# christoskokas/gtsam-vSLAM

Measured on AMD Instinct MI355X. Metric: frames/sec (extract+match+localBA), 1500 feat stereo 752x480, higher is better.
Workload: dtype u8/i32 (extract, match) + f64 (pose LM, local BA)

## Files before the change

gtsam-vslam_amd/csrc/ba.hip:

```cpp
#include "common.hpp"
#include "comm.hpp"
#include "dmath.hpp"
#include "ba_pool.hpp"
#include <algorithm>
#include <cmath>
#include <numeric>
#include <vector>
#include <atomic>
#include <condition_variable>
#include <functional>
#include <memory>
#include <mutex>
#include <thread>

namespace vslam {

struct BaEdge {
    int a, b, fa, fb;
    DPose measured;
    double r[6], Ja[36], Jb[36];
    double Haa[36], Hab[36], Hbb[36], ga[6], gb[6];
};

struct BaDev {
// ... 41 lines not shown
    D.poseCur = D.poseBase + (size_t)sel * D.K; D.poseTrial = D.poseBase + (size_t)ts * D.K;
    D.lmCur = D.lmBase + (size_t)sel * D.lmStride; D.lmTrial = D.lmBase + (size_t)ts * D.lmStride;
    if (D.specLin) {
        const size_t se = (size_t)D.n * D.n + D.n;
        D.facJ = D.facJBase + (size_t)sel * D.facJStride; D.facJ2 = D.facJBase + (size_t)ts * D.facJStride;
        D.Sedge = D.SedgeBase + (size_t)sel * se; D.Sedge2 = D.SedgeBase + (size_t)ts * se;
        D.edges = D.edgesBase + (size_t)sel * D.NE; D.edges2 = D.edgesBase + (size_t)ts * D.NE;
    }
    D.S += (size_t)c * D.sysStride; D.rhs += (size_t)c * D.sysStride; D.Spart += (size_t)c * D.spartStride;
    D.dP += (size_t)c * D.n; D.dL += (size_t)c * D.dLStride; D.partial += (size_t)c * D.partialStride;
    double lam = D.ctl[CTL_LAMBDA];
    for (int i = 0; i < c; i++) lam *= 10.0;
    D.lambda = lam;
    return true;
}

constexpr int BA_SCHUR_WAVES = 16;
constexpr int BA_LDS_MAX_F = 20;
constexpr int BA_LDS_BYTES = 160 * 1024, BA_STATIC_LDS_RESERVE = 1024, BA_DYN_LDS_MAX = BA_LDS_BYTES - BA_STATIC_LDS_RESERVE;

__device__ __forceinline__ void ba_eval_fac(const BaDev& D, const DPose& T, const double* p, bool right,
                                            const double* z, double is, double* r, double* Jp, double* Jl) {
    const double d[3] = {p[0] - T.t[0], p[1] - T.t[1], p[2] - T.t[2]};
    double q[3];
    mat3T_vec(T.R, d, q);
    if (Jp) { for (int c = 0; c < 12; c++) Jp[c] = 0; for (int c = 0; c < 6; c++) Jl[c] = 0; }
    if (is == 0.0) { r[0] = r[1] = 0.0; return; }
    if (q[2] <= 0) { r[0] = r[1] = 2.0 * D.fx * is; return; }
    const double x = q[0], y = q[1], zz = q[2], iz = 1.0 / zz;
    const double xx = right ? x - D.b : x;
// ... 182 lines not shown
    ci[CI_NACT] = D.NB;
}

__global__ __launch_bounds__(256) void k_ba_ctl(const BaDev* __restrict__ tab, int mode, double relTol, double absTol) {
    BaDev D = *lane_entry(tab, blockIdx.z);
    __shared__ int sZero;
    if (threadIdx.x == 0) {
        ba_ctl(D, mode, relTol, absTol);
        sZero = mode == 1 && ((const int*)(D.ctl + CTL_INTS))[CI_STATE] == BA_LINEARIZE;
    }
    __syncthreads();
    if (sZero) for (int i = threadIdx.x; i < D.n * D.n + D.n; i += 256) D.Sedge[i] = 0;
}

template <int MODE>
__global__ __launch_bounds__(256) void k_ba_factors(const BaDev* __restrict__ tab, int obsBlocks, int fuseCtl, double relTol, double absTol) {
    BaDev D = *lane_entry(tab, blockIdx.z);
    __shared__ double red[8], out[2];
    __shared__ double sW[160];
    __shared__ int sLast;
    double* const partialBase = D.partial;
    const int cand = MODE == 0 ? 0 : (int)blockIdx.y;
    const bool active = ba_enter(D, MODE == 0 ? BA_LINEARIZE : BA_TRY, cand);
    if (!active && ((const int*)(D.ctl + CTL_INTS))[CI_STATE] != (MODE == 0 ? BA_LINEARIZE : BA_TRY)) return;
    const int tid = threadIdx.x;
    if (!active) {
    } else if ((int)blockIdx.x < obsBlocks) {
        double v[2] = {0, 0};
        for (int f = blockIdx.x * 256 + tid; f < D.NF; f += obsBlocks * 256) {
            if (MODE == 0) {
                double r[2], Jp[12], Jl[6];
                ba_eval_fac(D, D.poseCur[D.facKf[f]], D.lmCur + 3 * (size_t)D.facLm[f], D.facRight[f], D.facZ + 2 * (size_t)f,
                            D.facIs[f], r, Jp, Jl);
                double* o = D.facJ + (size_t)f * 20;
                o[0] = r[0]; o[1] = r[1];
                for (int c = 0; c < 12; c++) o[2 + c] = Jp[c];
                for (int c = 0; c < 6; c++) o[14 + c] = Jl[c];
                v[0] += r[0] * r[0] + r[1] * r[1];
            } else {
                const double* o = D.facJ + (size_t)f * 20;
                const int fi = D.facFi[f], lp = D.facLp[f];
                double l0 = o[0], l1 = o[1];
                if (fi >= 0) {
                    const double* dp = D.dP + 6 * fi;
// ... 6 lines not shown
                if (D.specLin) {
                    double Jp[12], Jl[6];
                    ba_eval_fac(D, D.poseTrial[D.facKf[f]], D.lmTrial + 3 * (size_t)D.facLm[f], D.facRight[f], D.facZ + 2 * (size_t)f,
                                D.facIs[f], r, Jp, Jl);
                    double* o2 = D.facJ2 + (size_t)f * 20;
                    o2[0] = r[0]; o2[1] = r[1];
                    for (int c = 0; c < 12; c++) o2[2 + c] = Jp[c];
                    for (int c = 0; c < 6; c++) o2[14 + c] = Jl[c];
                } else
                    ba_eval_fac(D, D.poseTrial[D.facKf[f]], D.lmTrial + 3 * (size_t)D.facLm[f], D.facRight[f], D.facZ + 2 * (size_t)f,
                                D.facIs[f], r, nullptr, nullptr);
                v[1] += r[0] * r[0] + r[1] * r[1];
            }
        }
        ba_block_sum<2, 4>(v, red, out);
        if (tid == 0) { ba_publish(&D.partial[2 * blockIdx.x], out[0]); ba_publish(&D.partial[2 * blockIdx.x + 1], out[1]); }
    } else {
        const int e = blockIdx.x - obsBlocks;
        double v[2] = {0, 0};
        if (e < D.NE) {
            const BaEdge& E = D.edges[e];
            const int fa = E.fa, fb = E.fb;
            if (MODE == 0) {
                v[0] = ba_edge_linearize(D.edges[e], E, D.poseCur[E.a], D.poseCur[E.b], sW, D.Sedge, D.n, tid);
            } else {
                if (tid >= 8 && tid < 14) {
                    const int k = tid - 8;
                    double l = E.r[k];
                    for (int i = 0; i < 6; i++) {
                        if (fa >= 0) l += E.Ja[k * 6 + i] * D.dP[6 * fa + i];
                        if (fb >= 0) l += E.Jb[k * 6 + i] * D.dP[6 * fb + i];
                    }
                    v[0] += l * l;
// ... 6 lines not shown
                    pose_inverse(E.measured, Mi);
                    pose_compose(Mi, h, d);
                    double r[6];
                    pose3_logmap(d, r);
                    for (int i = 0; i < 6; i++) { r[i] *= 1.0 / 0.01; v[1] += r[i] * r[i]; }
                }
            }
#pragma unroll
            for (int k = 0; k < 2; k++) {
#pragma unroll
                for (int d = 32; d >= 1; d >>= 1) v[k] += __shfl_xor(v[k], d);
            }
            if (tid == 0) { ba_publish(&D.partial[2 * obsBlocks + 2 * e], v[0]); ba_publish(&D.partial[2 * obsBlocks + 2 * e + 1], v[1]); }
        }
    }
    asm volatile("s_waitcnt vmcnt(0)" ::: "memory");
    __syncthreads();
    const int nCandRun = MODE == 0 ? 1 : D.nAct;
    if (tid == 0) sLast = (__hip_atomic_fetch_add(&D.flags[FLAG_COUNT], 1, __ATOMIC_RELAXED, __HIP_MEMORY_SCOPE_AGENT) == (int)(gridDim.x * gridDim.y) - 1);
    __syncthreads();
    if (!sLast) return;
    const int nPart = obsBlocks + D.NE;
    for (int c = 0; c < nCandRun; c++) {
        const double* part = partialBase + (size_t)c * D.partialStride;
        double t[2] = {0, 0};
        for (int i = tid; i < nPart; i += 256) { t[0] += ba_collect(&part[2 * i]); t[1] += ba_collect(&part[2 * i + 1]); }
        ba_block_sum<2, 4>(t, red, out);
        if (tid == 0) {
            if (MODE == 0) D.sums[0] = 0.5 * out[0];
            else { D.sums[SUMS_CAND + 2 * c] = 0.5 * out[0]; D.sums[SUMS_CAND + 2 * c + 1] = 0.5 * out[1]; }
        }
        __syncthreads();
    }
    if (tid == 0) {
        D.flags[FLAG_COUNT] = 0;
        sLast = 0;
        if (fuseCtl) {
            ba_ctl(D, MODE, relTol, absTol);
            sLast = MODE == 1 && !D.specLin && ((const int*)(D.ctl + CTL_INTS))[CI_STATE] == BA_LINEARIZE;
            if (D.ctlHost) {
                asm volatile("s_waitcnt vmcnt(0) lgkmcnt(0)" ::: "memory");
// ... 43 lines not shown
        double acc = 0;
        for (int f = D.slotStart[s0 + s]; f < D.slotStart[s0 + s + 1]; f++) {
            const double* o = D.facJ + (size_t)f * 20;
            acc += o[2 + i] * o[14 + j] + o[2 + 6 + i] * o[14 + 3 + j];
        }
        W[e] = acc;
    }
    for (int s = lane; s < ns; s += BA_LPL) sfi[s] = D.slotFi[s0 + s];
}
__device__ __forceinline__ void ba_hll_inverse(const double* h, double lambda, double* Hi) {
    const double Hll[9] = {h[0] + lambda, h[1], h[2], h[1], h[3] + lambda, h[4], h[2], h[4], h[5] + lambda};
    inv3sym(Hll, Hi);
}

__global__ __launch_bounds__(64 * BA_SCHUR_WAVES) void k_ba_schur(const BaDev* __restrict__ tab, int maxSlots, int sharedW) {
    BaDev D = *lane_entry(tab, blockIdx.z);
    constexpr bool LDS_S = true;
    extern __shared__ double sm[];
    double* const SBase = D.S;
    double* const SpartBase = D.Spart;
    (void)SBase;
    const int c0 = sharedW ? 0 : (int)blockIdx.y;
    if (!ba_enter(D, BA_TRY, c0)) return;
    const int nc = sharedW ? D.nAct : 1;
    const int n = D.n;
    const size_t sys = (size_t)n * n + n;
    constexpr int BA_LPL = BA_LPL_SCHUR;
    double* Sloc = sm;
    double* wbase = sm + (LDS_S ? (size_t)nc * sys : 0);
    static_assert(BA_LPL == 64, "one wave per landmark: the landmark index is wave-uniform");
    const int lane = threadIdx.x & (BA_LPL - 1);
    const int unit = __builtin_amdgcn_readfirstlane(threadIdx.x / BA_LPL);
    double* W = wbase + (size_t)unit * (2 * maxSlots * 18);
    double* WH = W + maxSlots * 18;
    const int nu = blockDim.x / BA_LPL, nt = blockDim.x;
    int* sfi = (int*)(wbase + (size_t)nu * (2 * maxSlots * 18)) + unit * maxSlots;
    if (LDS_S) {
        for (int i = threadIdx.x; i < (int)(nc * sys); i += nt) Sloc[i] = 0;
    }
    __syncthreads();
    const int bi = lane / 6, bj = lane - bi * 6;
    const bool isBlk = lane < 36, isRhs = lane >= 36 && lane < 42;
    const int rr = isRhs ? lane - 36 : 0;
    const int hHalf = lane >= 27 ? 1 : 0, hq = lane - 27 * hHalf;
    const bool hRhs = hq >= 21;
    int hI = 0, hJ = 0;
    if (hRhs) hI = hq - 21;
    else { int rem = hq; while (rem >= 6 - hI) { rem -= 6 - hI; hI++; } hJ = hI + rem; }
    const int rounds = (D.Lp + gridDim.x * nu - 1) / (gridDim.x * nu);
    for (int rd = 0; rd < rounds; rd++) {
        const int lp = (rd * gridDim.x + blockIdx.x) * nu + unit;
        const bool act = lp < D.Lp;
        double h[9];
        int ns = 0;
        ba_lm_blocks<BA_LPL>(D, lp, act, W, sfi, h, ns);
        ba_wave_fence();
        double lamk = D.lambda;
        for (int k = 0; k < nc; k++, lamk *= 10.0) {
            double* Sacc = LDS_S ? Sloc + (size_t)k * sys : SBase + (size_t)(c0 + k) * D.sysStride;
            double* racc = Sacc + (size_t)n * n;
            double Hi[9];
            ba_hll_inverse(h, lamk, Hi);
            for (int e = lane; e < ns * 18; e += BA_LPL) {
                const int s = e / 18, ij = e - s * 18, i = ij / 3, j = ij - i * 3;
                const double* w = W + s * 18 + i * 3;
                WH[e] = w[0] * Hi[j] + w[1] * Hi[3 + j] + w[2] * Hi[6 + j];
// ... 18 lines not shown
        const int f0 = act ? D.lpStart[lp] : 0, f1 = act ? D.lpStart[lp + 1] : 0;
        if (lane < 54) {
            for (int f = f0 + hHalf; f < f1; f += 2) {
                const int fi = D.facFi[f];
                if (fi < 0) continue;
                const double* o = D.facJ + (size_t)f * 20;
                const double val = hRhs ? -(o[2 + hI] * o[0] + o[8 + hI] * o[1]) : o[2 + hI] * o[2 + hJ] + o[8 + hI] * o[8 + hJ];
                const size_t idx = hRhs ? (size_t)n * n + 6 * fi + hI : (size_t)(6 * fi + hI) * n + 6 * fi + hJ;
                for (int k = 0; k < nc; k++) atomicAdd((LDS_S ? Sloc + (size_t)k * sys : SBase + (size_t)(c0 + k) * D.sysStride) + idx, val);
            }
        }
    }
    if (LDS_S) {
        __syncthreads();
        for (int k = 0; k < nc; k++) {
            double* dst = SpartBase + (size_t)(c0 + k) * D.spartStride + (size_t)blockIdx.x * sys;
            for (int i = threadIdx.x; i < (int)sys; i += nt) dst[i] = Sloc[(size_t)k * sys + i];
        }
    }
}

constexpr int BA2_MAX_F = 10;
__host__ __device__ inline int ba2_stage_doubles(int maxFac, int maxSlots) {
    const int ints = maxFac + 2 * (maxSlots + 1);
    return ((maxFac * 20 + 2 * maxSlots * 18 + 10 + (ints + 1) / 2) + 1) & ~1;
}
__device__ __forceinline__ double ba2_dpp_xor(double v, int which) {
    const int lo = __double2loint(v), hi = __double2hiint(v);
    int l2, h2;
    if (which == 0) { l2 = __builtin_amdgcn_update_dpp(0, lo, 0xB1, 0xF, 0xF, true); h2 = __builtin_amdgcn_update_dpp(0, hi, 0xB1, 0xF, 0xF, true); }
    else { l2 = __builtin_amdgcn_update_dpp(0, lo, 0x4E, 0xF, 0xF, true); h2 = __builtin_amdgcn_update_dpp(0, hi, 0x4E, 0xF, 0xF, true); }
    return __hiloint2double(h2, l2);
}
// ... 45 lines not shown
#pragma unroll
    for (int k = 0; k < 9; k++) h[k] = g.hb[k];
}
__device__ __forceinline__ void ba2_w_row(const Ba2Region& g, const Ba2Roles& R, double& w0, double& w1, double& w2) {
    w0 = w1 = w2 = 0;
    for (int f = g.sst[R.ws]; f < g.sst[R.ws + 1]; f++) {
        const double* o = g.F + f * 20;
        const double a0 = o[2 + R.wi], a1 = o[8 + R.wi];
        w0 += a0 * o[14] + a1 * o[17];
        w1 += a0 * o[15] + a1 * o[18];
        w2 += a0 * o[16] + a1 * o[19];
    }
}

__global__ __launch_bounds__(1024) void k_ba_schur2(const BaDev* __restrict__ tab, int maxSlots, int maxFac) {
    BaDev D = *lane_entry(tab, blockIdx.z);
    extern __shared__ double sm[];
    if (!ba_enter(D, BA_TRY, blockIdx.y)) return;
    const int n = D.n;
    const int sys = n * n + n;
    double* const Sloc = sm;
    double* const racc = Sloc + (size_t)n * n;
    const int lane = threadIdx.x & 63;
    const int unit = __builtin_amdgcn_readfirstlane(threadIdx.x >> 6), nu = blockDim.x >> 6, nt = blockDim.x;
    const Ba2Region g = ba2_region(sm + sys + (size_t)unit * ba2_stage_doubles(maxFac, maxSlots), maxFac, maxSlots);
    double* const F = g.F; double* const W = g.W; double* const WH = g.WH;
    int* const ffi = g.ffi; int* const sfi = g.sfi;
    const double lam = D.lambda;
    Ba2Roles R;
    R.init(lane);
    const int pf = lane / 6, pi = lane - pf * 6;
    for (int i = threadIdx.x; i < sys; i += nt) Sloc[i] = 0;
    __syncthreads();
    for (int lp = blockIdx.x * nu + unit; lp < D.Lp; lp += gridDim.x * nu) {
        double h[9];
        int nf, ns;
        ba2_stage_h(D, lp, g, R, lane, h, nf, ns);
        double Hi[9];
        ba_hll_inverse(h, lam, Hi);
        if (R.ws < ns) {
            double w0, w1, w2;
            ba2_w_row(g, R, w0, w1, w2);
            const double g0 = w0 * Hi[0] + w1 * Hi[3] + w2 * Hi[6], g1 = w0 * Hi[1] + w1 * Hi[4] + w2 * Hi[7], g2 = w0 * Hi[2] + w1 * Hi[5] + w2 * Hi[8];
            double* wr = W + R.ws * 18 + R.wi * 3;
            wr[0] = w0; wr[1] = w1; wr[2] = w2;
            double* gr = WH + R.ws * 18 + R.wi * 3;
            gr[0] = g0; gr[1] = g1; gr[2] = g2;
            atomicAdd(&racc[6 * sfi[R.ws] + R.wi], -(g0 * h[6] + g1 * h[7] + g2 * h[8]));
        }
// ... 23 lines not shown
        if (pf < 10)
            for (int fb = 0; fb < nf; fb += 10) {
                const int f = fb + pf;
                if (f >= nf) break;
                const int fi = ffi[f];
                if (fi < 0) continue;
                const double* o = F + f * 20;
                const double a0 = o[2 + pi], a1 = o[8 + pi];
                double* dr = Sloc + (6 * fi + pi) * n + 6 * fi;
                for (int j = pi; j < 6; j++) atomicAdd(dr + j, a0 * o[2 + j] + a1 * o[8 + j]);
                atomicAdd(&racc[6 * fi + pi], -(a0 * o[0] + a1 * o[1]));
            }
        ba_wave_fence();
    }
    __syncthreads();
    double* dst = D.Spart + (size_t)blockIdx.x * sys;
    for (int i = threadIdx.x; i < sys; i += nt) dst[i] = Sloc[i];
}

__global__ __launch_bounds__(512) void k_ba_back2(const BaDev* __restrict__ tab, int maxSlots, int maxFac) {
    BaDev D = *lane_entry(tab, blockIdx.z);
    extern __shared__ double sm[];
    if (!ba_enter(D, BA_TRY, 0)) return;
    const int nc = D.nAct;
    const int sel = ((const int*)(D.ctl + CTL_INTS))[CI_SEL];
    const int lane = threadIdx.x & 63;
    const int unit = __builtin_amdgcn_readfirstlane(threadIdx.x >> 6), nu = blockDim.x >> 6;
    const Ba2Region g = ba2_region(sm + (size_t)unit * ba2_stage_doubles(maxFac, maxSlots), maxFac, maxSlots);
    Ba2Roles R;
    R.init(lane);
    for (int lp = blockIdx.x * nu + unit; lp < D.Lp; lp += gridDim.x * nu) {
        double h[9];
        int nf, ns;
        ba2_stage_h(D, lp, g, R, lane, h, nf, ns);
        double w0 = 0, w1 = 0, w2 = 0;
        int kcol = 0;
// ... 13 lines not shown
            if (lane < 3) {
                const double u0 = h[6] - t0, u1 = h[7] - t1, u2 = h[8] - t2;
                const double h0 = lane == 0 ? Hi[0] : (lane == 1 ? Hi[3] : Hi[6]);
                const double h1 = lane == 0 ? Hi[1] : (lane == 1 ? Hi[4] : Hi[7]);
                const double h2 = lane == 0 ? Hi[2] : (lane == 1 ? Hi[5] : Hi[8]);
                const double dl = h0 * u0 + h1 * u1 + h2 * u2;
                D.dL[(size_t)k * D.dLStride + 3 * (size_t)lp + lane] = dl;
                double* lmT = D.lmBase + (size_t)ba_slot(sel, k, D.NB) * D.lmStride;
                lmT[3 * (size_t)l + lane] = D.lmCur[3 * (size_t)l + lane] + dl;
            }
        }
        ba_wave_fence();
    }
}

__global__ __launch_bounds__(256) void k_ba_reduce(const BaDev* __restrict__ tab, int nPart) {
    BaDev D = *lane_entry(tab, blockIdx.z);
    __shared__ double sSl[8][33];
    if (!ba_enter(D, BA_TRY, blockIdx.y)) return;
    const int total = D.n * D.n + D.n;
    const int e = threadIdx.x & 31, y = threadIdx.x >> 5;
    const int i = blockIdx.x * 32 + e;
    const size_t stride = (size_t)total;
    double s = 0;
    if (i < total) {
        const int per = (nPart + 7) / 8;
        const int p0 = y * per, p1 = min(nPart, p0 + per);
        double s0 = 0, s1 = 0, s2 = 0, s3 = 0;
        int p = p0;
        for (; p + 3 < p1; p += 4) {
            s0 += D.Spart[(size_t)p * stride + i];
            s1 += D.Spart[(size_t)(p + 1) * stride + i];
            s2 += D.Spart[(size_t)(p + 2) * stride + i];
            s3 += D.Spart[(size_t)(p + 3) * stride + i];
        }
        for (; p < p1; p++) s0 += D.Spart[(size_t)p * stride + i];
        s = (s0 + s1) + (s2 + s3);
    }
    sSl[y][e] = s;
    __syncthreads();
    if (y == 0 && i < total) {
        double t = D.Sedge[i];
        for (int q = 0; q < 8; q++) t += sSl[q][e];
        if (D.specLin) D.Sedge2[i] = 0;
        if (i < D.n * D.n) D.S[i] = t; else D.rhs[i - D.n * D.n] = t;
    }
}

struct BaWin {
    int TB, T, TP, tileDoubles, nWin;
    const int* winA; const int* winB;
    const int* winFirstWg;
    const int* wgWin; const int* wgBegin; const int* wgEnd;
    const int* winLm;
    double* part;
    double* Wg; double* Hg;
};

constexpr int BA_WIN_HG = 9 + 6 * BA_MAX_NB;
__global__ __launch_bounds__(64 * BA_SCHUR_WAVES) void k_ba_lm_prep(const BaDev* __restrict__ tab, BaWin Wn, int maxSlots) {
// ... 307 lines not shown
        }
        BA_STAMP(5)
        for (int k = tid; k < D.K; k += nt) {
            const int fi = D.fidx[k];
            if (fi >= 0) { DPose T; pose_retract(D.poseCur[k], D.dP + 6 * fi, T); D.poseTrial[k] = T; }
            else D.poseTrial[k] = D.poseCur[k];
        }
    }
    __syncthreads();
    BA_STAMP(6)
    if (tid == 0) D.flags[FLAG_FAIL + D.cand] = sFail;
}

constexpr int BA_WAVE_N = 60;
__global__ __launch_bounds__(64) void k_ba_solve_wave(const BaDev* __restrict__ tab) {
    BaDev D = *lane_entry(tab, blockIdx.z);
    constexpr int N = BA_WAVE_N;
    __shared__ double Lt[N * (N + 1)];
    if (D.solveKind != BA_SOLVE_WAVE) return;
    if (!ba_enter(D, BA_TRY, blockIdx.x)) return;
    const double lambda = D.lambda;
    const int n = D.n, lane = threadIdx.x;
    const int r = lane < N ? lane : N - 1;
    double a[N];
#ifdef VSLAM_BA_STAMPS
#define BAW_STAMP(i) if (lane == 0) D.sums[8 + (i)] = (double)__builtin_readcyclecounter();
#else
#define BAW_STAMP(i)
#endif
    BAW_STAMP(0)
// ... 49 lines not shown
        asm volatile("s_waitcnt lgkmcnt(0)" ::: "memory");
        for (int k = lane; k < D.K; k += 64) {
            const int fi = D.fidx[k];
            if (fi >= 0) { DPose T; pose_retract(D.poseCur[k], Lt + 6 * fi, T); D.poseTrial[k] = T; }
            else D.poseTrial[k] = D.poseCur[k];
        }
    }
    BAW_STAMP(6)
    if (lane == 0) D.flags[FLAG_FAIL + D.cand] = bad ? 1 : 0;
}

constexpr int BA_MFMA_N = 256, BA_MFMA_NB = BA_MFMA_N / 16, BA_MFMA_NW = 8, BA_MFMA_SLOTS = 17, BA_MFMA_LD = 17;
typedef double ba_d4 __attribute__((ext_vector_type(4)));

__global__ __launch_bounds__(64 * BA_MFMA_NW) void k_ba_solve_mfma(const BaDev* __restrict__ tab, double* __restrict__ Lg) {
    BaDev D = *lane_entry(tab, blockIdx.z);
    extern __shared__ double sm[];
    double* P = sm;
    double* sInv = P + BA_MFMA_N * BA_MFMA_LD;
    double* sB = sInv + 16;
    __shared__ int sBad;
    if (D.solveKind != BA_SOLVE_MFMA) return;
    if (!ba_enter(D, BA_TRY, blockIdx.x)) return;
    const double lambda = D.lambda;
    constexpr int N = BA_MFMA_N, NB = BA_MFMA_NB, LD = BA_MFMA_LD;
    if (D.Lg) Lg = D.Lg;
    Lg += (size_t)D.cand * N * N;
    const int n = D.n, tid = threadIdx.x, lane = tid & 63;
    const int wave = __builtin_amdgcn_readfirstlane(tid >> 6);
    if (tid == 0) sBad = 0;
// ... 131 lines not shown
                sB[row] = v;
            }
            __syncthreads();
        }
        for (int i = tid; i < n; i += 64 * BA_MFMA_NW) D.dP[i] = sB[i];
        for (int k = tid; k < D.K; k += 64 * BA_MFMA_NW) {
            const int fi = D.fidx[k];
            if (fi >= 0) { DPose T; pose_retract(D.poseCur[k], sB + 6 * fi, T); D.poseTrial[k] = T; }
            else D.poseTrial[k] = D.poseCur[k];
        }
    }
    if (tid == 0) D.flags[FLAG_FAIL + D.cand] = fail ? 1 : 0;
}

__global__ __launch_bounds__(64) void k_ba_solve_mfma64(const BaDev* __restrict__ tab) {
    BaDev D = *lane_entry(tab, blockIdx.z);
    constexpr int N = 64, LDF = 65, LD = 17;
    __shared__ double Lf[N * LDF];
    __shared__ double P[N * LD];
    __shared__ double sInv[16], sB[N];
    if (D.solveKind != BA_SOLVE_MFMA64) return;
    if (!ba_enter(D, BA_TRY, blockIdx.x)) return;
    const double lambda = D.lambda;
    const int n = D.n, lane = threadIdx.x;
    auto fence = []() { asm volatile("s_waitcnt lgkmcnt(0)" ::: "memory"); };
    for (int row = 0; row < n; row++)
        if (lane < n) Lf[row * LDF + lane] = D.S[(size_t)row * n + lane];
    sB[lane] = lane < n ? D.rhs[lane] : 0.0;
    asm volatile("s_waitcnt vmcnt(0) lgkmcnt(0)" ::: "memory");
    ba_d4 acc[10];
// ... 318 lines not shown
                if (lane == k) b = xk; else if (lane < k) b = __builtin_fma(-lki, xk, b);
            }
            sX[J * CH_B + lane] = b;
        }
        __syncthreads();
    }
    for (int i = tid; i < n; i += 256) D.dP[i] = sX[i];
    for (int k = tid; k < D.K; k += 256) {
        const int fi = D.fidx[k];
        if (fi >= 0) { DPose T; pose_retract(D.poseCur[k], sX + 6 * fi, T); D.poseTrial[k] = T; }
        else D.poseTrial[k] = D.poseCur[k];
    }
}

__global__ __launch_bounds__(64 * BA_SCHUR_WAVES) void k_ba_back(const BaDev* __restrict__ tab, int maxSlots, int allCand) {
    BaDev D = *lane_entry(tab, blockIdx.z);
    extern __shared__ double sm[];
    const int c0 = allCand ? 0 : (int)blockIdx.y;
    if (!ba_enter(D, BA_TRY, c0)) return;
    const int nc = allCand ? D.nAct : 1;
    const int sel = ((const int*)(D.ctl + CTL_INTS))[CI_SEL];
    constexpr int BA_LPL = BA_LPL_BACK;
    const int lane = threadIdx.x & (BA_LPL - 1), unit = threadIdx.x / BA_LPL;
    double* W = sm + (size_t)unit * (maxSlots * 18);
    const int nu = blockDim.x / BA_LPL;
    int* sfi = (int*)(sm + (size_t)nu * (maxSlots * 18)) + unit * maxSlots;
    const int rounds = (D.Lp + gridDim.x * nu - 1) / (gridDim.x * nu);
    for (int rd = 0; rd < rounds; rd++) {
        const int lp = (rd * gridDim.x + blockIdx.x) * nu + unit;
        const bool act = lp < D.Lp;
        double h[9];
        int ns = 0;
        ba_lm_blocks<BA_LPL>(D, lp, act, W, sfi, h, ns);
        ba_wave_fence();
        const int l = act ? D.lpOrig[lp] : 0;
        double lamk = D.lambda;
        for (int k = 0; k < nc; k++, lamk *= 10.0) {
            const double* dPk = D.dP + (size_t)k * D.n;
            double Hi[9];
            ba_hll_inverse(h, lamk, Hi);
            double t[3] = {0, 0, 0};
            for (int e = lane; e < ns * 6; e += BA_LPL) {
                const int s = e / 6, i = e - s * 6;
                const double dp = dPk[6 * sfi[s] + i];
// ... 5 lines not shown
#pragma unroll
                for (int d = BA_LPL / 2; d >= 1; d >>= 1) t[q] += __shfl_xor(t[q], d);
            }
            if (act && lane < 3) {
                const double u[3] = {h[6] - t[0], h[7] - t[1], h[8] - t[2]};
                const double h0 = lane == 0 ? Hi[0] : (lane == 1 ? Hi[3] : Hi[6]);
                const double h1 = lane == 0 ? Hi[1] : (lane == 1 ? Hi[4] : Hi[7]);
                const double h2 = lane == 0 ? Hi[2] : (lane == 1 ? Hi[5] : Hi[8]);
                const double dl = h0 * u[0] + h1 * u[1] + h2 * u[2];
                D.dL[(size_t)k * D.dLStride + 3 * (size_t)lp + lane] = dl;
                double* lmT = D.lmBase + (size_t)ba_slot(sel, c0 + k, D.NB) * D.lmStride;
                lmT[3 * (size_t)l + lane] = D.lmCur[3 * (size_t)l + lane] + dl;
            }
        }
        ba_wave_fence();
    }
}

struct BaChi {
    int NP; const int* pairKf; const int* pairLm; const uint8_t* pairFlags; const float* pairUv; const int* pairOct;
    const uint8_t* kfLocal; const uint8_t* kfPresent; const uint8_t* lmPresent; const DPose* pose; const double* lm;
    float thr[MAX_LEVELS]; double fx, fy, cx, cy, b; uint8_t* wrong;
};
__device__ __forceinline__ bool ba_outlier(const BaChi& C, const double* pc, float ou, float ov, int oct, bool right) {
    const double x = right ? pc[0] - C.b : pc[0], y = pc[1], z = pc[2];
    if (z <= 0) return true;
    const double px = C.fx * x + C.cx * z, py = C.fy * y + C.cy * z;
    const double eu = (double)ou - px / z, ev = (double)ov - py / z;
    return (eu * eu + ev * ev) > (double)C.thr[oct];
}
// ... 1126 lines not shown
        *h_D = D;
        const BaDev* const dD = A.dev(h_D);
        VS_HIP(hipMemcpyAsync((void*)dD, h_D, sizeof(BaDev), hipMemcpyHostToDevice, stream));
        BHS("upload");

        auto run_lm = [&](int ps, long long nfStat, long long lpStat, long long k2Stat) -> vslam_status {
        (void)poseOut; (void)lmOut;
        const int fuseCtl = comm ? 0 : 1;
        const int facBlocks = (NF ? obsBlocks : 0) + std::max(NE, 1);
        const int nObs = NF ? obsBlocks : 0;
        VS_HIP(hipMemsetAsync(d_Sedge.p, 0, ((size_t)n * n + n) * sizeof(double), stream));
        auto step = [&](bool first) -> vslam_status {
            int t = -1;
            if (first || !specLin) {
                t = g_baTimer.begin("ba_linearize");
                hipLaunchKernelGGL(k_ba_factors<0>, dim3(facBlocks), dim3(256), 0, stream, dD, nObs, fuseCtl, relTol, absTol);
                g_baTimer.end(t);
            }
            if (comm) {
                const int tc = g_baTimer.begin("ba_allreduce"); VS_CHECK(comm_allreduce(comm, d_sums.p, 1, stream)); g_baTimer.end(tc);
                hipLaunchKernelGGL(k_ba_ctl, dim3(1), dim3(256), 0, stream, dD, 0, relTol, absTol);
            }
            t = g_baTimer.begin("ba_schur");
            if (n > 0) {
                if (ldsS) hipLaunchKernelGGL(k_ba_schur, dim3(lmBlocks, sharedW ? 1 : NB), dim3(64 * schurWaves), schurLds, stream, dD, maxSlots, sharedW);
                else if (nWinWg) {
                    hipLaunchKernelGGL(k_ba_lm_prep, dim3(std::max(1, std::min((Lp + BA_SCHUR_WAVES - 1) / BA_SCHUR_WAVES, 4 * nCU))), dim3(64 * BA_SCHUR_WAVES),
                                       (size_t)BA_SCHUR_WAVES * maxSlots * sizeof(int), stream, dD, Wn, maxSlots);
                    hipLaunchKernelGGL(k_ba_schur_win, dim3(nWinWg), dim3(64 * schurWaves), schurLds, stream, dD, Wn);
                }
            }
            g_baTimer.end(t);
            t = g_baTimer.begin("ba_solve");
            if (n > 0) {
                if (ldsS) hipLaunchKernelGGL(k_ba_reduce, dim3(((int)sysDoubles + 31) / 32, NB), dim3(256), 0, stream, dD, lmBlocks);
                else hipLaunchKernelGGL(k_ba_reduce_win, dim3(Wn.nWin, NB), dim3(256), 0, stream, dD, Wn);
            }
            if (comm && n > 0) { const int tc = g_baTimer.begin("ba_allreduce"); VS_CHECK(comm_allreduce(comm, d_S.p, sysStride * (NB - 1) + (size_t)n * n + n, stream)); g_baTimer.end(tc); }
            if (n <= 64 && useMfma) hipLaunchKernelGGL(k_ba_solve_mfma64, dim3(NB), dim3(64), 0, stream, dD);
            else if (n <= BA_WAVE_N) hipLaunchKernelGGL(k_ba_solve_wave, dim3(NB), dim3(64), 0, stream, dD);
            else if (n <= BA_MFMA_N && useMfma) hipLaunchKernelGGL(k_ba_solve_mfma, dim3(NB), dim3(64 * BA_MFMA_NW), mfmaLds, stream, dD, d_Lg.p);
            else if (useChol) {
                for (int J = 0; J < cholN / CH_B; J++)
                    hipLaunchKernelGGL(k_ba_chol_col, dim3(cholN / CH_B - J, NB), dim3(256), cholColLds, stream, dD, d_Lg.p, d_cholY.p, cholN, J, d_cholFail.p);
                hipLaunchKernelGGL(k_ba_chol_back, dim3(NB), dim3(256), cholBackLds, stream, dD, (const double*)d_Lg.p, (const double*)d_cholY.p, cholN, d_cholFail.p);
            } else hipLaunchKernelGGL(k_ba_solve, dim3(NB), dim3(std::max(64, vslam::align_up(n, 64))),
                                    solveLds ? solveLdsBytes : 64, stream, dD, solveLds ? 1 : 0, solveLds ? ldA : n);
            g_baTimer.end(t);
            t = g_baTimer.begin("ba_back");
            if (Lp) hipLaunchKernelGGL(k_ba_back, dim3(backBlocks, sharedBack ? 1 : NB), dim3(64 * backWaves), backLds, stream, dD, maxSlots, sharedBack);
            g_baTimer.end(t);
            t = g_baTimer.begin("ba_eval");
            hipLaunchKernelGGL(k_ba_factors<1>, dim3(facBlocks, NB), dim3(256), 0, stream, dD, nObs, fuseCtl, relTol, absTol);
            g_baTimer.end(t);
            if (comm) {
                const int tc = g_baTimer.begin("ba_allreduce"); VS_CHECK(comm_allreduce(comm, d_sums.p + SUMS_CAND, (size_t)2 * NB, stream)); g_baTimer.end(tc);
                hipLaunchKernelGGL(k_ba_ctl, dim3(1), dim3(256), 0, stream, dD, 1, relTol, absTol);
            }
            VS_HIP(hipGetLastError());
            return VSLAM_OK;
        };
        double* h_ctlOut = ws->h_ctlOut;
        const int* co = (const int*)(h_ctlOut + CTL_INTS);
        int enq = 0;
        for (;;) {
            static const int perPoll = getenv("VSLAM_BA_STEPS_PER_POLL") ? std::max(1, atoi(getenv("VSLAM_BA_STEPS_PER_POLL"))) : 4;
            for (int b = 0; b < perPoll; b++) VS_CHECK(step(enq + b == 0));
            enq += perPoll;
// ... 369 lines not shown
        q.H.fill(P, q.wrong.data(), 0, 1, q.T, q.pose0.data(), nullptr, nSlots);
        ba_init_ctl(q.H.h_ctl, 0, adaptive ? 1 : NB);
    });
    BBS(1);
    int nMax = 0, neMax = 0, nfMax = 0, npMax = 0, valMax = 0;
    for (int i : act) {
        const Lane& q = lanes[i];
        nMax = std::max(nMax, q.H.n); neMax = std::max(neMax, q.H.NE);
        nfMax = std::max(nfMax, q.H.NF); npMax = std::max(npMax, q.NP);
        valMax = std::max(valMax, std::max(q.K * (int)(sizeof(DPose) / sizeof(double)), 3 * q.L));
    }
    plan_cohort();
    const vslam_ba_batch_plan& plan = g_baLastPlan;
    if (plan.status != VSLAM_OK) { set_error("local BA batch: landmark with too many views for the LDS staging"); return VSLAM_ERR_CAPACITY; }
    const int nCU = 256;
    const int obsBlocks = std::max(1, std::min((nfMax + 255) / 256, std::max(16, 2 * nCU / NL)));
    const int facBlocks = obsBlocks + std::max(neMax, 1);
    const size_t sysMax = (size_t)nMax * nMax + nMax;
    const int maxSlots = plan.max_slots, maxFac = plan.max_factors, lmBlocks = plan.schur_blocks;
    const bool useSchur2 = plan.schur_kernel == VSLAM_BA_KERNEL_SCHUR2, useBack2 = plan.back_kernel == VSLAM_BA_KERNEL_BACK2;
    const bool anyMfma64 = plan.solve_kinds & (1 << BA_SOLVE_MFMA64), anyWave = plan.solve_kinds & (1 << BA_SOLVE_WAVE),
               anyMfma = plan.solve_kinds & (1 << BA_SOLVE_MFMA);
    VS_CHECK(ba_kernel_attributes());
    size_t dBytes = 0;
    auto dtake = [&](size_t bytes) { const size_t at = dBytes; dBytes = (dBytes + std::max<size_t>(bytes, 8) + 255) & ~(size_t)255; return at; };
    struct Off { size_t flags, sedge, poseS, lmS, facJ, dP, dL, S, partial, spart, sums, Lg, wrong, outPose, outLm; };
    std::vector<Off> off(NL);
    for (int a = 0; a < NL; a++) { const Lane& q = lanes[act[a]]; off[a].flags = dtake(16 * sizeof(int)); off[a].sedge = dtake(((size_t)q.H.n * q.H.n + q.H.n) * nSlots * 8); }
    const size_t zeroBytes = dBytes;
    size_t wrongBase = 0, wrongEnd = 0, outBase = 0, outEnd = 0;
    wrongBase = dBytes;
// ... 64 lines not shown
        X.nPose = K * (int)(sizeof(DPose) / sizeof(double)); X.nLm = 3 * L; X.pose0 = (const double*)A.dev(q.h_pose0); X.lm0 = A.dev(q.h_lm0);
        X.outPose = q.d_outPose; X.outLm = q.d_outLm;
        h_aux[a] = X;
    }
    const BaDev* const dTab = A.dev(h_tab);
    const BaLaneAux* const dAux = A.dev(h_aux);
    VS_HIP(A.upload(stream));
    VS_HIP(hipMemsetAsync(dm, 0, zeroBytes, stream));
    const int valBlocks = std::max(1, std::min((valMax + 255) / 256, 64));
    hipLaunchKernelGGL(k_ba_init_slots_b, dim3(valBlocks, NL), dim3(256), 0, stream, dTab, dAux);

    auto step = [&](bool first) -> vslam_status {
        int t = -1;
        if (first) {
            t = g_baTimer.begin("ba_linearize");
            hipLaunchKernelGGL(k_ba_factors<0>, dim3(facBlocks, 1, NL), dim3(256), 0, stream, dTab, obsBlocks, 1, relTol, absTol);
            g_baTimer.end(t);
        }
        t = g_baTimer.begin("ba_schur");
        if (useSchur2) hipLaunchKernelGGL(k_ba_schur2, dim3(lmBlocks, NB, NL), dim3(64 * plan.schur_waves), plan.schur_lds, stream, dTab, maxSlots, maxFac);
        else hipLaunchKernelGGL(k_ba_schur, dim3(lmBlocks, plan.schur_shared_w ? 1 : NB, NL), dim3(64 * plan.schur_waves), plan.schur_lds, stream, dTab, maxSlots, plan.schur_shared_w);
        g_baTimer.end(t);
        t = g_baTimer.begin("ba_solve");
        hipLaunchKernelGGL(k_ba_reduce, dim3(((int)sysMax + 31) / 32, NB, NL), dim3(256), 0, stream, dTab, lmBlocks);
        if (anyMfma64) hipLaunchKernelGGL(k_ba_solve_mfma64, dim3(NB, 1, NL), dim3(64), 0, stream, dTab);
        if (anyWave) hipLaunchKernelGGL(k_ba_solve_wave, dim3(NB, 1, NL), dim3(64), 0, stream, dTab);
        if (anyMfma) hipLaunchKernelGGL(k_ba_solve_mfma, dim3(NB, 1, NL), dim3(64 * BA_MFMA_NW), plan.solve_lds, stream, dTab, (double*)nullptr);
        g_baTimer.end(t);
        t = g_baTimer.begin("ba_back");
        if (useBack2) hipLaunchKernelGGL(k_ba_back2, dim3(plan.back_blocks, 1, NL), dim3(64 * plan.back_waves), plan.back_lds, stream, dTab, maxSlots, maxFac);
        else hipLaunchKernelGGL(k_ba_back, dim3(plan.back_blocks, plan.back_shared ? 1 : NB, NL), dim3(64 * plan.back_waves), plan.back_lds, stream, dTab, maxSlots, plan.back_shared);
        g_baTimer.end(t);
        t = g_baTimer.begin("ba_eval");
        hipLaunchKernelGGL(k_ba_factors<1>, dim3(facBlocks, NB, NL), dim3(256), 0, stream, dTab, obsBlocks, 1, relTol, absTol);
        g_baTimer.end(t);
        VS_HIP(hipGetLastError());
        return VSLAM_OK;
    };
    double* const b_ctl = (double*)(W.h_back + oBackCtl);
    memcpy(b_ctl, h_ctlAll, (size_t)CTL_DOUBLES * 8 * NL);
    auto lm_loop = [&](int first) -> vslam_status {
        static const int perPollEnv = getenv("VSLAM_BA_STEPS_PER_POLL") ? std::max(1, atoi(getenv("VSLAM_BA_STEPS_PER_POLL"))) : 0;
        int enq = 0, polls = 0;
        for (;;) {
            const int batch = perPollEnv ? perPollEnv : (enq == 0 ? first : 2);
            for (int b = 0; b < batch; b++) VS_CHECK(step(enq + b == 0));
            enq += batch;
            static const bool mirrorOff = getenv("VSLAM_BA_CTL_MIRROR") && atoi(getenv("VSLAM_BA_CTL_MIRROR")) == 0;
            if (mirrorOff || ++polls > 4) VS_HIP(hipMemcpyAsync(b_ctl, A.dev(h_ctlAll), (size_t)CTL_DOUBLES * 8 * NL, hipMemcpyDeviceToHost, stream));
// ... 302 lines not shown
```

Baseline: 29270.

## Fold LM candidates into x-grid slices and early-exit idle candidate blocks

Changes the batched local-BA kernels (factors eval, schur, reduce, back) so that, by default, candidate lambdas are not spread over gridDim.y. Instead each x-block is assigned one candidate and a slice of the landmark/observation range, driven by the runtime active-candidate count. The per-candidate partial reductions are re-indexed to match. It also adds early-return checks on the control state and candidate count before the full descriptor is copied, so blocks for inactive candidates exit cheaply. This cuts wasted launch slots when adaptive mode runs only one candidate, at the cost of more complex indexing and less parallelism per candidate when many are active.

```diff
diff --git a/gtsam-vslam_amd/csrc/ba.hip b/gtsam-vslam_amd/csrc/ba.hip
--- a/gtsam-vslam_amd/csrc/ba.hip
+++ b/gtsam-vslam_amd/csrc/ba.hip
@@ -79,6 +79,23 @@
     D.lambda = lam;
     return true;
 }
+__device__ __forceinline__ bool ba_due(const BaDev* E, int state, int y = 0) {
+    const int* ci = (const int*)(E->ctl + CTL_INTS);
+    return ci[CI_STATE] == state && y < ci[CI_NACT];
+}
+struct BaCandPlan { int j0, j1, si, ns; };
+__device__ __forceinline__ BaCandPlan ba_cand_plan(int nAct, int y, int gy, int x, int nx) {
+    const int nMine = y < nAct ? (nAct - y + gy - 1) / gy : 0;
+    BaCandPlan p;
+    if (nMine > 0 && nx >= nMine) { p.j0 = x % nMine; p.j1 = p.j0 + 1; p.si = x / nMine; p.ns = (nx - p.j0 + nMine - 1) / nMine; }
+    else { p.j0 = 0; p.j1 = nMine; p.si = x; p.ns = nx; }
+    return p;
+}
+__device__ __forceinline__ int ba_cand_slices(int nAct, int c, int gy, int nx) {
+    if (gy <= 0) return nx;
+    const int y = c % gy, j = c / gy, nMine = (nAct - y + gy - 1) / gy;
+    return nx >= nMine ? (nx - j + nMine - 1) / nMine : nx;
+}
 
 constexpr int BA_SCHUR_WAVES = 16;
 constexpr int BA_LDS_MAX_F = 20;
@@ -291,20 +308,32 @@
 }
 
 template <int MODE>
-__global__ __launch_bounds__(256) void k_ba_factors(const BaDev* __restrict__ tab, int obsBlocks, int fuseCtl, double relTol, double absTol) {
-    BaDev D = *lane_entry(tab, blockIdx.z);
+__global__ __launch_bounds__(256) void k_ba_factors(const BaDev* __restrict__ tab, int obsBlocks, int fuseCtl, double relTol, double absTol, int edgeCand) {
+    const BaDev* const ent = lane_entry(tab, blockIdx.z);
     __shared__ double red[8], out[2];
     __shared__ double sW[160];
     __shared__ int sLast;
-    double* const partialBase = D.partial;
-    const int cand = MODE == 0 ? 0 : (int)blockIdx.y;
-    const bool active = ba_enter(D, MODE == 0 ? BA_LINEARIZE : BA_TRY, cand);
-    if (!active && ((const int*)(D.ctl + CTL_INTS))[CI_STATE] != (MODE == 0 ? BA_LINEARIZE : BA_TRY)) return;
-    const int tid = threadIdx.x;
+    const int* const ci0 = (const int*)(ent->ctl + CTL_INTS);
+    if (ci0[CI_STATE] != (MODE == 0 ? BA_LINEARIZE : BA_TRY)) return;
+    const int nCandRun = MODE == 0 ? 1 : __builtin_amdgcn_readfirstlane(ci0[CI_NACT]);
+    const int tid = threadIdx.x, gy = gridDim.y;
+    const bool isObs = (int)blockIdx.x < obsBlocks;
+    BaCandPlan cp = {0, 1, isObs ? (int)blockIdx.x : 0, isObs ? obsBlocks : 1};
+    int edge = (int)blockIdx.x - obsBlocks;
+    if (MODE == 1) {
+        if (isObs) cp = ba_cand_plan(nCandRun, blockIdx.y, gy, blockIdx.x, obsBlocks);
+        else {
+            const int nMine = (int)blockIdx.y < nCandRun ? (nCandRun - (int)blockIdx.y + gy - 1) / gy : 0;
+            cp.j0 = edge % edgeCand; cp.j1 = cp.j0 < nMine ? cp.j0 + 1 : cp.j0;
+            edge /= edgeCand;
+        }
+    }
+    BaDev D = *ent;
+    const bool active = cp.j0 < cp.j1 && ba_enter(D, MODE == 0 ? BA_LINEARIZE : BA_TRY, (int)blockIdx.y + gy * cp.j0);
     if (!active) {
-    } else if ((int)blockIdx.x < obsBlocks) {
+    } else if (isObs) {
         double v[2] = {0, 0};
-        for (int f = blockIdx.x * 256 + tid; f < D.NF; f += obsBlocks * 256) {
+        for (int f = cp.si * 256 + tid; f < D.NF; f += cp.ns * 256) {
             if (MODE == 0) {
                 double r[2], Jp[12], Jl[6];
                 ba_eval_fac(D, D.poseCur[D.facKf[f]], D.lmCur + 3 * (size_t)D.facLm[f], D.facRight[f], D.facZ + 2 * (size_t)f,
@@ -341,9 +370,9 @@
             }
         }
         ba_block_sum<2, 4>(v, red, out);
-        if (tid == 0) { ba_publish(&D.partial[2 * blockIdx.x], out[0]); ba_publish(&D.partial[2 * blockIdx.x + 1], out[1]); }
+        if (tid == 0) { ba_publish(&D.partial[2 * cp.si], out[0]); ba_publish(&D.partial[2 * cp.si + 1], out[1]); }
     } else {
-        const int e = blockIdx.x - obsBlocks;
+        const int e = edge;
         double v[2] = {0, 0};
         if (e < D.NE) {
             const BaEdge& E = D.edges[e];
@@ -380,17 +409,20 @@
             if (tid == 0) { ba_publish(&D.partial[2 * obsBlocks + 2 * e], v[0]); ba_publish(&D.partial[2 * obsBlocks + 2 * e + 1], v[1]); }
         }
     }
+    double* const partialBase = ent->partial;
     asm volatile("s_waitcnt vmcnt(0)" ::: "memory");
     __syncthreads();
-    const int nCandRun = MODE == 0 ? 1 : D.nAct;
     if (tid == 0) sLast = (__hip_atomic_fetch_add(&D.flags[FLAG_COUNT], 1, __ATOMIC_RELAXED, __HIP_MEMORY_SCOPE_AGENT) == (int)(gridDim.x * gridDim.y) - 1);
     __syncthreads();
     if (!sLast) return;
-    const int nPart = obsBlocks + D.NE;
     for (int c = 0; c < nCandRun; c++) {
         const double* part = partialBase + (size_t)c * D.partialStride;
+        const int nObsPart = ba_cand_slices(nCandRun, c, gy, obsBlocks), nPart = nObsPart + D.NE;
         double t[2] = {0, 0};
-        for (int i = tid; i < nPart; i += 256) { t[0] += ba_collect(&part[2 * i]); t[1] += ba_collect(&part[2 * i + 1]); }
+        for (int i = tid; i < nPart; i += 256) {
+            const int q = i < nObsPart ? i : obsBlocks + (i - nObsPart);
+            t[0] += ba_collect(&part[2 * q]); t[1] += ba_collect(&part[2 * q + 1]);
+        }
         ba_block_sum<2, 4>(t, red, out);
         if (tid == 0) {
             if (MODE == 0) D.sums[0] = 0.5 * out[0];
@@ -464,13 +496,19 @@
 }
 
 __global__ __launch_bounds__(64 * BA_SCHUR_WAVES) void k_ba_schur(const BaDev* __restrict__ tab, int maxSlots, int sharedW) {
-    BaDev D = *lane_entry(tab, blockIdx.z);
+    const BaDev* const ent = lane_entry(tab, blockIdx.z);
+    if (!ba_due(ent, BA_TRY, sharedW ? 0 : (int)blockIdx.y)) return;
     constexpr bool LDS_S = true;
     extern __shared__ double sm[];
+    const int nActRound = ((const int*)(ent->ctl + CTL_INTS))[CI_NACT];
+    BaCandPlan cp = {0, 1, (int)blockIdx.x, (int)gridDim.x};
+    if (!sharedW) cp = ba_cand_plan(nActRound, blockIdx.y, gridDim.y, blockIdx.x, gridDim.x);
+    for (int cj = cp.j0; cj < cp.j1; cj++) {
+    BaDev D = *ent;
     double* const SBase = D.S;
     double* const SpartBase = D.Spart;
     (void)SBase;
-    const int c0 = sharedW ? 0 : (int)blockIdx.y;
+    const int c0 = sharedW ? 0 : (int)blockIdx.y + (int)gridDim.y * cj;
     if (!ba_enter(D, BA_TRY, c0)) return;
     const int nc = sharedW ? D.nAct : 1;
     const int n = D.n;
@@ -497,9 +535,9 @@
     int hI = 0, hJ = 0;
     if (hRhs) hI = hq - 21;
     else { int rem = hq; while (rem >= 6 - hI) { rem -= 6 - hI; hI++; } hJ = hI + rem; }
-    const int rounds = (D.Lp + gridDim.x * nu - 1) / (gridDim.x * nu);
+    const int rounds = (D.Lp + cp.ns * nu - 1) / (cp.ns * nu);
     for (int rd = 0; rd < rounds; rd++) {
-        const int lp = (rd * gridDim.x + blockIdx.x) * nu + unit;
+        const int lp = (rd * cp.ns + cp.si) * nu + unit;
         const bool act = lp < D.Lp;
         double h[9];
         int ns = 0;
@@ -548,9 +586,11 @@
     if (LDS_S) {
         __syncthreads();
         for (int k = 0; k < nc; k++) {
-            double* dst = SpartBase + (size_t)(c0 + k) * D.spartStride + (size_t)blockIdx.x * sys;
+            double* dst = SpartBase + (size_t)(c0 + k) * D.spartStride + (size_t)cp.si * sys;
             for (int i = threadIdx.x; i < (int)sys; i += nt) dst[i] = Sloc[(size_t)k * sys + i];
         }
+        __syncthreads();
+    }
     }
 }
 
@@ -626,9 +666,13 @@
 }
 
 __global__ __launch_bounds__(1024) void k_ba_schur2(const BaDev* __restrict__ tab, int maxSlots, int maxFac) {
-    BaDev D = *lane_entry(tab, blockIdx.z);
+    const BaDev* const ent = lane_entry(tab, blockIdx.z);
+    if (!ba_due(ent, BA_TRY, blockIdx.y)) return;
     extern __shared__ double sm[];
-    if (!ba_enter(D, BA_TRY, blockIdx.y)) return;
+    const BaCandPlan cp = ba_cand_plan(((const int*)(ent->ctl + CTL_INTS))[CI_NACT], blockIdx.y, gridDim.y, blockIdx.x, gridDim.x);
+    for (int cj = cp.j0; cj < cp.j1; cj++) {
+    BaDev D = *ent;
+    if (!ba_enter(D, BA_TRY, (int)blockIdx.y + (int)gridDim.y * cj)) return;
     const int n = D.n;
     const int sys = n * n + n;
     double* const Sloc = sm;
@@ -644,7 +688,7 @@
     const int pf = lane / 6, pi = lane - pf * 6;
     for (int i = threadIdx.x; i < sys; i += nt) Sloc[i] = 0;
     __syncthreads();
-    for (int lp = blockIdx.x * nu + unit; lp < D.Lp; lp += gridDim.x * nu) {
+    for (int lp = cp.si * nu + unit; lp < D.Lp; lp += cp.ns * nu) {
         double h[9];
         int nf, ns;
         ba2_stage_h(D, lp, g, R, lane, h, nf, ns);
@@ -698,12 +742,16 @@
         ba_wave_fence();
     }
     __syncthreads();
-    double* dst = D.Spart + (size_t)blockIdx.x * sys;
+    double* dst = D.Spart + (size_t)cp.si * sys;
     for (int i = threadIdx.x; i < sys; i += nt) dst[i] = Sloc[i];
+    if (cj + 1 < cp.j1) __syncthreads();
+    }
 }
 
 __global__ __launch_bounds__(512) void k_ba_back2(const BaDev* __restrict__ tab, int maxSlots, int maxFac) {
-    BaDev D = *lane_entry(tab, blockIdx.z);
+    const BaDev* const ent = lane_entry(tab, blockIdx.z);
+    if (!ba_due(ent, BA_TRY)) return;
+    BaDev D = *ent;
     extern __shared__ double sm[];
     if (!ba_enter(D, BA_TRY, 0)) return;
     const int nc = D.nAct;
@@ -747,10 +795,15 @@
     }
 }
 
-__global__ __launch_bounds__(256) void k_ba_reduce(const BaDev* __restrict__ tab, int nPart) {
-    BaDev D = *lane_entry(tab, blockIdx.z);
+__global__ __launch_bounds__(256) void k_ba_reduce(const BaDev* __restrict__ tab, int nSlices, int schurGy) {
+    const BaDev* const ent = lane_entry(tab, blockIdx.z);
+    if (!ba_due(ent, BA_TRY, blockIdx.y)) return;
     __shared__ double sSl[8][33];
-    if (!ba_enter(D, BA_TRY, blockIdx.y)) return;
+    const int nActRound = ((const int*)(ent->ctl + CTL_INTS))[CI_NACT];
+    for (int c = blockIdx.y; c < nActRound; c += gridDim.y) {
+    BaDev D = *ent;
+    if (!ba_enter(D, BA_TRY, c)) return;
+    const int nPart = ba_cand_slices(nActRound, c, schurGy, nSlices);
     const int total = D.n * D.n + D.n;
     const int e = threadIdx.x & 31, y = threadIdx.x >> 5;
     const int i = blockIdx.x * 32 + e;
@@ -777,6 +830,8 @@
         for (int q = 0; q < 8; q++) t += sSl[q][e];
         if (D.specLin) D.Sedge2[i] = 0;
         if (i < D.n * D.n) D.S[i] = t; else D.rhs[i - D.n * D.n] = t;
+    }
+    __syncthreads();
     }
 }
 
@@ -1114,6 +1169,7 @@
 
 constexpr int BA_WAVE_N = 60;
 __global__ __launch_bounds__(64) void k_ba_solve_wave(const BaDev* __restrict__ tab) {
+    if (!ba_due(lane_entry(tab, blockIdx.z), BA_TRY, blockIdx.x)) return;
     BaDev D = *lane_entry(tab, blockIdx.z);
     constexpr int N = BA_WAVE_N;
     __shared__ double Lt[N * (N + 1)];
@@ -1193,6 +1249,7 @@
 typedef double ba_d4 __attribute__((ext_vector_type(4)));
 
 __global__ __launch_bounds__(64 * BA_MFMA_NW) void k_ba_solve_mfma(const BaDev* __restrict__ tab, double* __restrict__ Lg) {
+    if (!ba_due(lane_entry(tab, blockIdx.z), BA_TRY, blockIdx.x)) return;
     BaDev D = *lane_entry(tab, blockIdx.z);
     extern __shared__ double sm[];
     double* P = sm;
@@ -1354,6 +1411,7 @@
 }
 
 __global__ __launch_bounds__(64) void k_ba_solve_mfma64(const BaDev* __restrict__ tab) {
+    if (!ba_due(lane_entry(tab, blockIdx.z), BA_TRY, blockIdx.x)) return;
     BaDev D = *lane_entry(tab, blockIdx.z);
     constexpr int N = 64, LDF = 65, LD = 17;
     __shared__ double Lf[N * LDF];
@@ -1702,9 +1760,14 @@
 }
 
 __global__ __launch_bounds__(64 * BA_SCHUR_WAVES) void k_ba_back(const BaDev* __restrict__ tab, int maxSlots, int allCand) {
-    BaDev D = *lane_entry(tab, blockIdx.z);
+    const BaDev* const ent = lane_entry(tab, blockIdx.z);
+    if (!ba_due(ent, BA_TRY, allCand ? 0 : (int)blockIdx.y)) return;
     extern __shared__ double sm[];
-    const int c0 = allCand ? 0 : (int)blockIdx.y;
+    BaCandPlan cp = {0, 1, (int)blockIdx.x, (int)gridDim.x};
+    if (!allCand) cp = ba_cand_plan(((const int*)(ent->ctl + CTL_INTS))[CI_NACT], blockIdx.y, gridDim.y, blockIdx.x, gridDim.x);
+    for (int cj = cp.j0; cj < cp.j1; cj++) {
+    BaDev D = *ent;
+    const int c0 = allCand ? 0 : (int)blockIdx.y + (int)gridDim.y * cj;
     if (!ba_enter(D, BA_TRY, c0)) return;
     const int nc = allCand ? D.nAct : 1;
     const int sel = ((const int*)(D.ctl + CTL_INTS))[CI_SEL];
@@ -1713,9 +1776,9 @@
     double* W = sm + (size_t)unit * (maxSlots * 18);
     const int nu = blockDim.x / BA_LPL;
     int* sfi = (int*)(sm + (size_t)nu * (maxSlots * 18)) + unit * maxSlots;
-    const int rounds = (D.Lp + gridDim.x * nu - 1) / (gridDim.x * nu);
+    const int rounds = (D.Lp + cp.ns * nu - 1) / (cp.ns * nu);
     for (int rd = 0; rd < rounds; rd++) {
-        const int lp = (rd * gridDim.x + blockIdx.x) * nu + unit;
+        const int lp = (rd * cp.ns + cp.si) * nu + unit;
         const bool act = lp < D.Lp;
         double h[9];
         int ns = 0;
@@ -1751,6 +1814,7 @@
             }
         }
         ba_wave_fence();
+    }
     }
 }
 
@@ -2907,7 +2971,7 @@
             int t = -1;
             if (first || !specLin) {
                 t = g_baTimer.begin("ba_linearize");
-                hipLaunchKernelGGL(k_ba_factors<0>, dim3(facBlocks), dim3(256), 0, stream, dD, nObs, fuseCtl, relTol, absTol);
+                hipLaunchKernelGGL(k_ba_factors<0>, dim3(facBlocks), dim3(256), 0, stream, dD, nObs, fuseCtl, relTol, absTol, 1);
                 g_baTimer.end(t);
             }
             if (comm) {
@@ -2926,7 +2990,7 @@
             g_baTimer.end(t);
             t = g_baTimer.begin("ba_solve");
             if (n > 0) {
-                if (ldsS) hipLaunchKernelGGL(k_ba_reduce, dim3(((int)sysDoubles + 31) / 32, NB), dim3(256), 0, stream, dD, lmBlocks);
+                if (ldsS) hipLaunchKernelGGL(k_ba_reduce, dim3(((int)sysDoubles + 31) / 32, NB), dim3(256), 0, stream, dD, lmBlocks, sharedW ? 0 : NB);
                 else hipLaunchKernelGGL(k_ba_reduce_win, dim3(Wn.nWin, NB), dim3(256), 0, stream, dD, Wn);
             }
             if (comm && n > 0) { const int tc = g_baTimer.begin("ba_allreduce"); VS_CHECK(comm_allreduce(comm, d_S.p, sysStride * (NB - 1) + (size_t)n * n + n, stream)); g_baTimer.end(tc); }
@@ -2944,7 +3008,7 @@
             if (Lp) hipLaunchKernelGGL(k_ba_back, dim3(backBlocks, sharedBack ? 1 : NB), dim3(64 * backWaves), backLds, stream, dD, maxSlots, sharedBack);
             g_baTimer.end(t);
             t = g_baTimer.begin("ba_eval");
-            hipLaunchKernelGGL(k_ba_factors<1>, dim3(facBlocks, NB), dim3(256), 0, stream, dD, nObs, fuseCtl, relTol, absTol);
+            hipLaunchKernelGGL(k_ba_factors<1>, dim3(facBlocks, NB), dim3(256), 0, stream, dD, nObs, fuseCtl, relTol, absTol, 1);
             g_baTimer.end(t);
             if (comm) {
                 const int tc = g_baTimer.begin("ba_allreduce"); VS_CHECK(comm_allreduce(comm, d_sums.p + SUMS_CAND, (size_t)2 * NB, stream)); g_baTimer.end(tc);
@@ -3344,7 +3408,9 @@
     const vslam_ba_batch_plan& plan = g_baLastPlan;
     if (plan.status != VSLAM_OK) { set_error("local BA batch: landmark with too many views for the LDS staging"); return VSLAM_ERR_CAPACITY; }
     const int nCU = 256;
-    const int obsBlocks = std::max(1, std::min((nfMax + 255) / 256, std::max(16, 2 * nCU / NL)));
+    static const bool candRowsEnv = getenv("VSLAM_BA_CAND_ROWS") && atoi(getenv("VSLAM_BA_CAND_ROWS")) != 0;
+    const int candGy = candRowsEnv ? NB : 1, edgeCand = candRowsEnv ? 1 : NB;
+    const int obsBlocks = std::max(edgeCand, std::min((nfMax + 255) / 256, std::max(16, 2 * nCU / NL)));
     const int facBlocks = obsBlocks + std::max(neMax, 1);
     const size_t sysMax = (size_t)nMax * nMax + nMax;
     const int maxSlots = plan.max_slots, maxFac = plan.max_factors, lmBlocks = plan.schur_blocks;
@@ -3439,25 +3505,25 @@
         int t = -1;
         if (first) {
             t = g_baTimer.begin("ba_linearize");
-            hipLaunchKernelGGL(k_ba_factors<0>, dim3(facBlocks, 1, NL), dim3(256), 0, stream, dTab, obsBlocks, 1, relTol, absTol);
+            hipLaunchKernelGGL(k_ba_factors<0>, dim3(facBlocks, 1, NL), dim3(256), 0, stream, dTab, obsBlocks, 1, relTol, absTol, 1);
             g_baTimer.end(t);
         }
         t = g_baTimer.begin("ba_schur");
-        if (useSchur2) hipLaunchKernelGGL(k_ba_schur2, dim3(lmBlocks, NB, NL), dim3(64 * plan.schur_waves), plan.schur_lds, stream, dTab, maxSlots, maxFac);
-        else hipLaunchKernelGGL(k_ba_schur, dim3(lmBlocks, plan.schur_shared_w ? 1 : NB, NL), dim3(64 * plan.schur_waves), plan.schur_lds, stream, dTab, maxSlots, plan.schur_shared_w);
+        if (useSchur2) hipLaunchKernelGGL(k_ba_schur2, dim3(lmBlocks, candGy, NL), dim3(64 * plan.schur_waves), plan.schur_lds, stream, dTab, maxSlots, maxFac);
+        else hipLaunchKernelGGL(k_ba_schur, dim3(lmBlocks, plan.schur_shared_w ? 1 : candGy, NL), dim3(64 * plan.schur_waves), plan.schur_lds, stream, dTab, maxSlots, plan.schur_shared_w);
         g_baTimer.end(t);
         t = g_baTimer.begin("ba_solve");
-        hipLaunchKernelGGL(k_ba_reduce, dim3(((int)sysMax + 31) / 32, NB, NL), dim3(256), 0, stream, dTab, lmBlocks);
+        hipLaunchKernelGGL(k_ba_reduce, dim3(((int)sysMax + 31) / 32, candGy, NL), dim3(256), 0, stream, dTab, lmBlocks, !useSchur2 && plan.schur_shared_w ? 0 : candGy);
         if (anyMfma64) hipLaunchKernelGGL(k_ba_solve_mfma64, dim3(NB, 1, NL), dim3(64), 0, stream, dTab);
         if (anyWave) hipLaunchKernelGGL(k_ba_solve_wave, dim3(NB, 1, NL), dim3(64), 0, stream, dTab);
         if (anyMfma) hipLaunchKernelGGL(k_ba_solve_mfma, dim3(NB, 1, NL), dim3(64 * BA_MFMA_NW), plan.solve_lds, stream, dTab, (double*)nullptr);
         g_baTimer.end(t);
         t = g_baTimer.begin("ba_back");
         if (useBack2) hipLaunchKernelGGL(k_ba_back2, dim3(plan.back_blocks, 1, NL), dim3(64 * plan.back_waves), plan.back_lds, stream, dTab, maxSlots, maxFac);
-        else hipLaunchKernelGGL(k_ba_back, dim3(plan.back_blocks, plan.back_shared ? 1 : NB, NL), dim3(64 * plan.back_waves), plan.back_lds, stream, dTab, maxSlots, plan.back_shared);
+        else hipLaunchKernelGGL(k_ba_back, dim3(plan.back_blocks, plan.back_shared ? 1 : candGy, NL), dim3(64 * plan.back_waves), plan.back_lds, stream, dTab, maxSlots, plan.back_shared);
         g_baTimer.end(t);
         t = g_baTimer.begin("ba_eval");
-        hipLaunchKernelGGL(k_ba_factors<1>, dim3(facBlocks, NB, NL), dim3(256), 0, stream, dTab, obsBlocks, 1, relTol, absTol);
+        hipLaunchKernelGGL(k_ba_factors<1>, dim3(obsBlocks + edgeCand * std::max(neMax, 1), candGy, NL), dim3(256), 0, stream, dTab, obsBlocks, 1, relTol, absTol, edgeCand);
         g_baTimer.end(t);
         VS_HIP(hipGetLastError());
         return VSLAM_OK;
```

Result: no change. 29350 (median of 5 runs) (+0.3%).
